# zyc00/Point-SAM

Hardware: AMD Instinct MI355X
Metric: point-clouds/sec (encode+1-prompt decode) (higher is better)
Workload: dtype f32 (fp32 in/out/accumulate; large GEMMs as row-scaled 2-way fp16 split x 3 MFMA products, fp32-grade error)

## Files before the change

point_sam_amd/build.py:

```python
import os
import subprocess
import sys
from concurrent.futures import ThreadPoolExecutor

CSRC = os.path.join(os.path.dirname(os.path.abspath(__file__)), "csrc")
LIB = os.path.join(CSRC, "libpointsam_hip.so")
HIPCC = os.environ.get("HIPCC", "/opt/rocm/bin/hipcc")
ARCH = "gfx950"
COMMON = ["--offload-arch=" + ARCH, "-O3", "-std=c++17", "-fPIC", "-fvisibility=hidden", "-Wall", "-Wno-unused-function"]
EXPERIMENTS = os.environ.get("PSAM_BUILD_EXPERIMENTS", "0") == "1"
SOURCES = [
    ("tokenizer.hip", ["-ffp-contract=off"]),
    ("gemm.hip", []),
    ("gemm_split.hip", []),
    ("gemm_f16x3p.hip", []),
    ("gemm_f16x3pp.hip", []),
    ("attention.hip", []),
    ("rowops.hip", []),
    ("blocks.hip", []),
    ("masks.hip", []),
    ("error.cpp", ["-x", "hip"]),
] + ([("experiments/gemm_f16x3q.hip", ["-I" + CSRC]), ("experiments/gemm_f16x3s.hip", ["-I" + CSRC]), ("experiments/gemm_f16x3c.hip", ["-I" + CSRC]),
        ("experiments/twoway.hip", ["-I" + CSRC])] if EXPERIMENTS else [])
if EXPERIMENTS:
    COMMON = COMMON + ["-DPSAM_BUILD_EXPERIMENTS"]
FLAGS_STAMP = os.path.join(CSRC, ".build_flags")
PROBE_SRC = os.path.join(CSRC, "probe", "mfma_probe.hip")
PROBE_LIB = os.path.join(CSRC, "probe", "libpsam_probe.so")


def _stale(out, deps):
    return not os.path.exists(out) or any(os.path.getmtime(d) > os.path.getmtime(out) for d in deps)


def build_library(force: bool = False, verbose: bool = False) -> str:
    hdrs = [os.path.join(CSRC, f) for f in sorted(os.listdir(CSRC)) if f.endswith(".h")]
    hdrs.append(os.path.join(os.path.dirname(os.path.dirname(CSRC)), "include", "pointsam_hip.h"))
    flags = " ".join(COMMON)
    if (open(FLAGS_STAMP).read() != flags) if os.path.exists(FLAGS_STAMP) else EXPERIMENTS:
        force = True
    jobs = []
    for src, extra in SOURCES:
        s = os.path.join(CSRC, src)
        o = os.path.join(CSRC, os.path.splitext(src)[0] + ".o")
        if force or _stale(o, [s, os.path.abspath(__file__)] + hdrs):
            jobs.append([HIPCC] + COMMON + extra + ["-c", s, "-o", o])
    def run(cmd):
        if verbose:
            print(" ".join(cmd), flush=True)
        r = subprocess.run(cmd, capture_output=True, text=True)
        if r.returncode != 0:
            raise RuntimeError("hipcc failed:\n" + " ".join(cmd) + "\n" + r.stderr)
        return r.stderr
    with ThreadPoolExecutor(max_workers=4) as ex:
        list(ex.map(run, jobs))
    objs = [os.path.join(CSRC, os.path.splitext(s)[0] + ".o") for s, _ in SOURCES]
    if force or jobs or _stale(LIB, objs):
        tmp = LIB + ".unlinted"
        run([HIPCC, "--offload-arch=" + ARCH, "-shared", "-fPIC", "-o", tmp] + objs)
        try:
            from . import isa_lint
        except ImportError:
            sys.path.insert(0, os.path.dirname(os.path.abspath(__file__)))
            import isa_lint
        bad = isa_lint.lint(tmp)
        if bad:
            os.replace(tmp, LIB + ".rejected")
            raise RuntimeError("libpointsam_hip.so contains packed-FP32 instructions with a non-uniform op_sel (see point_sam_amd/isa_lint.py):\n" +
                               "\n".join(f"  {k}: {i}" for k, i in bad))
        os.replace(tmp, LIB)
        with open(FLAGS_STAMP, "w") as f:
            f.write(flags)
    if force or _stale(PROBE_LIB, [PROBE_SRC]):
        run([HIPCC, "--offload-arch=" + ARCH, "-O3", "-std=c++17", "-fPIC", "-shared", "-o", PROBE_LIB, PROBE_SRC])
    return LIB


if __name__ == "__main__":
    print(build_library(force="--force" in sys.argv, verbose=True))
```

point_sam_amd/csrc/attention.hip:

```cpp
#include "common.h"
#include <math.h>
#include <utility>
#include <cstdlib>

typedef float f32x16 __attribute__((ext_vector_type(16)));
typedef float f32x4 __attribute__((ext_vector_type(4)));

constexpr int FA_BQ = 128;
constexpr int FA_BKV = 64;

struct FlashArgs {
    const float* q; const float* k; const float* v; float* o;
    int64_t ldq, ldk, ldv, ldo, sq, sk, sv, so;
    int H, Lq, Lk, B;
    float scale_log2e;
    const float* a_scale; float* o_scale; float k1, k2;
    int hd;
    int ksplit; float* sk_part; int* sk_count;
#ifdef PSAM_ATTN_ABLATE
    int abl;
#endif
};
#ifdef PSAM_ATTN_ABLATE
#define FA_ABL(bit) (p.abl & (bit))
// ... 336 lines not shown
        for (int s = 0; s < KSA; ++s)
#pragma unroll
            for (int e = 0; e < 2; ++e) {
                t[s][e] = (ok && s * 16 + h * 8 + e * 4 < hd) ? *reinterpret_cast<const f32x4*>(qp + s * 16 + e * 4) : f32x4{0.f, 0.f, 0.f, 0.f};
                amax = fmaxf(fmaxf(amax, fmaxf(fabsf(t[s][e][0]), fabsf(t[s][e][1]))), fmaxf(fabsf(t[s][e][2]), fabsf(t[s][e][3])));
            }
        amax = fmaxf(amax, __shfl_xor(amax, 32, 64));
        const float sq = f16_row_scale(amax);
        q_inv = fa_inv_pow2(sq);
#pragma unroll
        for (int s = 0; s < KSA; ++s) {
            unsigned hi[4], lo[4];
#pragma unroll
            for (int e = 0; e < 2; ++e) {
                fa_split2(fa_f32x2{t[s][e][0], t[s][e][1]} * sq, hi[2 * e], lo[2 * e]);
                fa_split2(fa_f32x2{t[s][e][2], t[s][e][3]} * sq, hi[2 * e + 1], lo[2 * e + 1]);
            }
            qh[s] = __builtin_bit_cast(fa_f16x8, fa_u32x4{hi[0], hi[1], hi[2], hi[3]});
            ql[s] = __builtin_bit_cast(fa_f16x8, fa_u32x4{lo[0], lo[1], lo[2], lo[3]});
        }
    }

    publish_max(0);
    __syncthreads();
    tile_scales(0, sk_cur, sv_cur);
    store_tile(0, sk_cur, sv_cur);
    __syncthreads();
    for (int t = t_first; t < ntiles; ++t) {
        const int buf = (t - t_first) & 1;
        const unsigned char* st_base = smem + buf * STAGE;
        if (t + 1 < ntiles && !FA_ABL(2)) load_tile((t + 1) * FA_BKV);
        const float c_s = p.scale_log2e * q_inv * fa_inv_pow2(sk_cur);
#pragma unroll
        for (int kt = 0; kt < FA_BKV / 32; ++kt) {
            const int key_base = t * FA_BKV + kt * 32;
            if (key_base >= p.Lk) break;
            f32x16 st;
#pragma unroll
            for (int r = 0; r < 16; ++r) st[r] = 0.f;
            const int krow = kt * 32 + r32;
            const unsigned char* kb = st_base + krow * KROW;
#pragma unroll
            for (int s = 0; s < KSA; ++s) {
                const int off = ((2 * s + h) ^ ((krow >> 1) & KSW)) << 4;
                const fa_f16x8 kh = *reinterpret_cast<const fa_f16x8*>(kb + off);
                const fa_f16x8 kl = *reinterpret_cast<const fa_f16x8*>(kb + KPLANE + off);
                if (FA_ABL(8)) { st[0] += (float)kh[0] + (float)kl[1]; continue; }
                st = __builtin_amdgcn_mfma_f32_32x32x16_f16(kh, ql[s], st, 0, 0, 0);
                st = __builtin_amdgcn_mfma_f32_32x32x16_f16(kl, qh[s], st, 0, 0, 0);
                st = __builtin_amdgcn_mfma_f32_32x32x16_f16(kh, qh[s], st, 0, 0, 0);
            }
            if (key_base + 32 > p.Lk) {
#pragma unroll
                for (int r = 0; r < 16; ++r)
                    if (key_base + (r & 3) + 8 * (r >> 2) + 4 * h >= p.Lk) st[r] = -INFINITY;
            }
            float mx = -INFINITY;
#pragma unroll
            for (int r = 0; r < 16; ++r) mx = fmaxf(mx, st[r]);
            mx = fmaxf(mx, __shfl_xor(mx, 32, 64)) * c_s;
            const float m_new = fmaxf(m_run, mx);
            const float alpha = __builtin_amdgcn_exp2f(m_run - m_new);
            const float m14 = m_new - 14.f;
            float ps = 0.f;
#pragma unroll
            for (int r = 0; r < 16; ++r) {
                st[r] = FA_ABL(4) ? __builtin_fmaf(st[r], c_s, -m14) : __builtin_amdgcn_exp2f(__builtin_fmaf(st[r], c_s, -m14));
                ps += st[r];
            }
            l_run = l_run * alpha + ps;
            m_run = m_new;
            const float fo = alpha * (sv_cur * fa_inv_pow2(sv_acc));
            sv_acc = sv_cur;
            if (__builtin_amdgcn_ballot_w64(fo != 1.f) != 0) {
#pragma unroll
                for (int d = 0; d < DT; ++d)
#pragma unroll
                    for (int r = 0; r < 16; ++r) oacc[d][r] *= fo;
            }
            fa_f16x8 ph[2], pl[2];
#pragma unroll
            for (int s2 = 0; s2 < 2; ++s2) {
                unsigned hi[4], lo[4];
#pragma unroll
                for (int e = 0; e < 4; ++e) {
                    if (FA_ABL(4)) { hi[e] = __builtin_bit_cast(unsigned, st[8 * s2 + 2 * e]); lo[e] = __builtin_bit_cast(unsigned, st[8 * s2 + 2 * e + 1]); }
                    else fa_split2(fa_f32x2{st[8 * s2 + 2 * e], st[8 * s2 + 2 * e + 1]}, hi[e], lo[e]);
                }
                ph[s2] = __builtin_bit_cast(fa_f16x8, fa_u32x4{hi[0], hi[1], hi[2], hi[3]});
                pl[s2] = __builtin_bit_cast(fa_f16x8, fa_u32x4{lo[0], lo[1], lo[2], lo[3]});
            }
#pragma unroll
            for (int s2 = 0; s2 < 2; ++s2)
#pragma unroll
                for (int d = 0; d < DTA; ++d) {
                    const int vrow = d * 32 + r32;
                    const unsigned char* vb = st_base + 2 * KPLANE + vrow * ROWB + (((kt * 4 + s2 * 2 + h) ^ ((vrow >> 1) & 7)) << 4);
                    const fa_f16x8 vh = *reinterpret_cast<const fa_f16x8*>(vb);
                    const fa_f16x8 vl = *reinterpret_cast<const fa_f16x8*>(vb + VPLANE);
                    if (FA_ABL(16)) { oacc[d][0] += (float)vh[0] + (float)vl[1] + (float)pl[s2][0] + (float)ph[s2][1]; continue; }
                    oacc[d] = __builtin_amdgcn_mfma_f32_32x32x16_f16(vh, pl[s2], oacc[d], 0, 0, 0);
                    oacc[d] = __builtin_amdgcn_mfma_f32_32x32x16_f16(vl, ph[s2], oacc[d], 0, 0, 0);
                    oacc[d] = __builtin_amdgcn_mfma_f32_32x32x16_f16(vh, ph[s2], oacc[d], 0, 0, 0);
                }
        }
        if (t + 1 < ntiles && !FA_ABL(1)) {
            publish_max(buf ^ 1);
            __syncthreads();
            tile_scales(buf ^ 1, sk_cur, sv_cur);
            store_tile(buf ^ 1, sk_cur, sv_cur);
        }
        if (!FA_ABL(32)) __syncthreads();
    }

    float l_tot = l_run + __shfl_xor(l_run, 32, 64);
    if (p.ksplit > 1) {
        constexpr int SC1 = 16, QUADS = DT * 4, SPLIT_BYTES = (QUADS * 256 + 128) * 16;
        const __amdgpu_buffer_rsrc_t rs = __builtin_amdgcn_make_buffer_rsrc((void*)(p.sk_part + (int64_t)bid * p.ksplit * (SPLIT_BYTES / 4)), 0, 0x7fffffff, 0x00020000);
        const float isv = fa_inv_pow2(sv_acc);
#pragma unroll
        for (int d = 0; d < DT; ++d)
#pragma unroll
            for (int r4 = 0; r4 < 4; ++r4) {
                const float a0 = oacc[d][4 * r4] * isv, a1 = oacc[d][4 * r4 + 1] * isv, a2 = oacc[d][4 * r4 + 2] * isv, a3 = oacc[d][4 * r4 + 3] * isv;
                const f32x4 vf = {a0, a1, a2, a3};
                __builtin_amdgcn_raw_buffer_store_b128(__builtin_bit_cast(fa_u32x4, vf), rs, split * SPLIT_BYTES + ((d * 4 + r4) * 256 + tid) * 16, 0, SC1);
            }
        {
            const fa_f32x2 ml = {m_run, l_tot};
            __builtin_amdgcn_raw_buffer_store_b64(__builtin_bit_cast(fa_u32x2, ml), rs, split * SPLIT_BYTES + QUADS * 256 * 16 + tid * 8, 0, SC1);
        }
        asm volatile("s_waitcnt vmcnt(0)" ::: "memory");
        __syncthreads();
        int* flag = reinterpret_cast<int*>(&smax[0][0][0]);
        if (tid == 0) *flag = (int)__hip_atomic_fetch_add(p.sk_count + bid, 1, __ATOMIC_RELAXED, __HIP_MEMORY_SCOPE_AGENT);
        __syncthreads();
        if (*flag != p.ksplit - 1) return;
        if (tid == 0) __hip_atomic_store(p.sk_count + bid, 0, __ATOMIC_RELAXED, __HIP_MEMORY_SCOPE_AGENT);
        float ms[4], ls[4], m_all = -INFINITY;
#pragma unroll
        for (int sp = 0; sp < 4; ++sp) {
            ms[sp] = -INFINITY; ls[sp] = 0.f;
            if (sp < p.ksplit) {
                const fa_f32x2 ml = __builtin_bit_cast(fa_f32x2, __builtin_amdgcn_raw_buffer_load_b64(rs, sp * SPLIT_BYTES + QUADS * 256 * 16 + tid * 8, 0, SC1));
                ms[sp] = ml[0]; ls[sp] = ml[1];
                m_all = fmaxf(m_all, ml[0]);
            }
        }
#pragma unroll
        for (int d = 0; d < DT; ++d)
#pragma unroll
            for (int r = 0; r < 16; ++r) oacc[d][r] = 0.f;
        l_tot = 0.f;
#pragma unroll
        for (int sp = 0; sp < 4; ++sp) {
            if (sp < p.ksplit) {
                const float w = __builtin_amdgcn_exp2f(ms[sp] - m_all);
                l_tot = __builtin_fmaf(w, ls[sp], l_tot);
#pragma unroll
                for (int d = 0; d < DT; ++d)
#pragma unroll
                    for (int r4 = 0; r4 < 4; ++r4) {
                        const f32x4 v = __builtin_bit_cast(f32x4, __builtin_amdgcn_raw_buffer_load_b128(rs, sp * SPLIT_BYTES + ((d * 4 + r4) * 256 + tid) * 16, 0, SC1));
#pragma unroll
                        for (int e = 0; e < 4; ++e) oacc[d][4 * r4 + e] = __builtin_fmaf(w, v[e], oacc[d][4 * r4 + e]);
                    }
            }
        }
        sv_acc = 1.f;
    }
    const float inv = fa_inv_pow2(sv_acc) / l_tot;
    const int qrow = q0 + r32;
    if (p.o_scale) {
        if (head == 0 && h == 0 && qrow < p.Lq) p.o_scale[(int64_t)b * p.Lq + qrow] = out_scale;
        float* op = p.o + b * p.so + (int64_t)(qrow < p.Lq ? qrow : 0) * p.ldo + head * hd;
#pragma unroll
        for (int d = 0; d < DT; ++d)
#pragma unroll
            for (int g = 0; g < 4; ++g) {
                const int d0 = d * 32 + 8 * g + 4 * h;
                unsigned h0, l0, h1, l1;
                fa_split2(fa_f32x2{oacc[d][4 * g] * inv, oacc[d][4 * g + 1] * inv} * out_scale, h0, l0);
                fa_split2(fa_f32x2{oacc[d][4 * g + 2] * inv, oacc[d][4 * g + 3] * inv} * out_scale, h1, l1);
                const unsigned r0 = __shfl_xor(h ? h0 : l0, 32, 64), r1 = __shfl_xor(h ? h1 : l1, 32, 64);
                if (qrow < p.Lq && d0 < hd) *reinterpret_cast<fa_u32x4*>(op + d0) = h ? fa_u32x4{r0, r1, l0, l1} : fa_u32x4{h0, h1, r0, r1};
            }
        return;
    }
    if (qrow < p.Lq) {
        float* op = p.o + b * p.so + (int64_t)qrow * p.ldo + head * hd;
#pragma unroll
        for (int d = 0; d < DT; ++d)
#pragma unroll
            for (int g = 0; g < 4; ++g) {
                const int d0 = d * 32 + 8 * g + 4 * h;
                f32x4 o4 = {oacc[d][4 * g] * inv, oacc[d][4 * g + 1] * inv, oacc[d][4 * g + 2] * inv, oacc[d][4 * g + 3] * inv};
                if (d0 < hd) *reinterpret_cast<f32x4*>(op + d0) = o4;
            }
    }
}

constexpr int64_t FA_SK_MAX_UNITS = PSAM_CNT_ATTN_N;
static int g_fa_keysplit = -1;
static bool fa_keysplit_enabled() {
    if (g_fa_keysplit >= 0) return g_fa_keysplit != 0;
    static int on = -1;
    if (on < 0) { const char* e = getenv("PSAM_ATTN_KEYSPLIT"); on = e ? (atoi(e) != 0) : 1; }
    return on != 0;
}
PSAM_API void psam_attention_f16x3_force_keysplit(int32_t mode) { g_fa_keysplit = mode; }
static bool fa_full_width() {
    static int on = -1;
    if (on < 0) { const char* e = getenv("PSAM_ATTN_FULL_WIDTH"); on = e ? (atoi(e) != 0) : 0; }
    return on != 0;
}
static int fa_keysplit_factor(int32_t B, int32_t H, int32_t Lq, int32_t Lk, int32_t hd, int32_t max_keysplit) {
    if (B <= 0 || H <= 0 || Lq <= 0 || Lk <= 0 || hd <= 64) return 1;
    const int64_t units = (int64_t)psam_cdiv(Lq, FA_BQ) * H * B;
    int dev = 0, ncu = 256;
    if (hipGetDevice(&dev) != hipSuccess || hipDeviceGetAttribute(&ncu, hipDeviceAttributeMultiprocessorCount, dev) != hipSuccess || ncu <= 0) ncu = 256;
    const int ntiles = (int)psam_cdiv(Lk, FA_BKV);
    int ks = fa_keysplit_enabled() ? (int)(ncu / units) : 1;
    if (ks > 4) ks = 4;
    if (ks > max_keysplit) ks = max_keysplit;
    if (ks > ntiles / 2) ks = ntiles / 2;
    return (ks > 1 && units <= FA_SK_MAX_UNITS) ? ks : 1;
}
static int64_t fa_split_bytes(int32_t hd) { return ((int64_t)((hd == 64 ? 64 : 128) / 32) * 4 * 256 + 128) * 16; }
PSAM_API size_t psam_attention_f16x3_keysplit_ws_bytes(int32_t B, int32_t H, int32_t Lq, int32_t Lk, int32_t hd, int32_t max_keysplit) {
    const int ks = fa_keysplit_factor(B, H, Lq, Lk, hd, max_keysplit);
    return ks > 1 ? (size_t)((int64_t)psam_cdiv(Lq, FA_BQ) * H * B * ks * fa_split_bytes(hd)) : 0;
}

PSAM_API int32_t psam_attention_f16x3_ex2(const float* q, int64_t ldq, int64_t sq, const float* k, int64_t ldk, int64_t sk, const float* v, int64_t ldv,
                                          int64_t sv, float* o, int64_t ldo, int64_t so, int32_t B, int32_t H, int32_t Lq, int32_t Lk, int32_t hd,
                                          float scale, const float* a_scale, float k1, float k2, float* o_scale, int32_t max_keysplit, void* ks_ws,
                                          size_t ks_ws_bytes, int32_t* counters, hipStream_t stream) {
    PSAM_REQUIRE(q && k && v && o, PSAM_EINVAL, "psam_attention_f16x3: null pointer");
    PSAM_REQUIRE((a_scale == nullptr) == (o_scale == nullptr), PSAM_EINVAL, "psam_attention_f16x3: packed output needs both a_scale and o_scale");
    PSAM_REQUIRE(!o_scale || ((ldo & 7) == 0 && ((uintptr_t)o & 31) == 0 && (so & 7) == 0 && Lq == Lk), PSAM_EINVAL,
                 "psam_attention_f16x3: packed output needs 32-byte aligned rows and self-attention (Lq == Lk)");
    PSAM_REQUIRE(B > 0 && H > 0 && Lq > 0 && Lk > 0, PSAM_EINVAL, "psam_attention_f16x3: bad shape");
    PSAM_REQUIRE((int64_t)psam_cdiv(Lq, FA_BQ) * H * B < ((int64_t)1 << 31), PSAM_EINVAL, "psam_attention_f16x3: too many workgroups");
    PSAM_REQUIRE(((ldq | ldk | ldv | ldo | sq | sk | sv | so) & 3) == 0 && (((uintptr_t)q | (uintptr_t)k | (uintptr_t)v | (uintptr_t)o) & 15) == 0,
                 PSAM_EALIGN, "psam_attention_f16x3: strides must be multiples of 4 floats and pointers 16-byte aligned");
    PSAM_REQUIRE((int64_t)Lk * ldk < ((int64_t)1 << 29) && (int64_t)Lk * ldv < ((int64_t)1 << 29), PSAM_EINVAL,
                 "psam_attention_f16x3: one (batch) K/V slice must span < 2 GiB (32-bit buffer offsets)");
    FlashArgs p;
    p.q = q; p.k = k; p.v = v; p.o = o;
    p.ldq = ldq; p.ldk = ldk; p.ldv = ldv; p.ldo = ldo; p.sq = sq; p.sk = sk; p.sv = sv; p.so = so;
    p.H = H; p.Lq = Lq; p.Lk = Lk; p.B = B;
    p.scale_log2e = scale * 1.4426950408889634f;
    p.a_scale = a_scale; p.o_scale = o_scale; p.k1 = k1; p.k2 = k2; p.hd = hd;
#ifdef PSAM_ATTN_ABLATE
    p.abl = g_attn_abl;
#endif
    p.ksplit = 1; p.sk_part = nullptr; p.sk_count = nullptr;
    const int64_t units = (int64_t)psam_cdiv(Lq, FA_BQ) * H * B;
    if (ks_ws && counters) {
        int ks = fa_keysplit_factor(B, H, Lq, Lk, hd, max_keysplit);
        while (ks > 1 && (size_t)(units * ks * fa_split_bytes(hd)) > ks_ws_bytes) --ks;
        if (ks > 1) {
            PSAM_REQUIRE(((uintptr_t)ks_ws & 15) == 0, PSAM_EALIGN, "psam_attention_f16x3: ks_ws must be 16-byte aligned");
            p.ksplit = ks; p.sk_part = static_cast<float*>(ks_ws); p.sk_count = counters + PSAM_CNT_ATTN;
        }
    }
    const dim3 grid((unsigned)(units * p.ksplit)), block(256);
    if (hd == 64) hipLaunchKernelGGL((flash_attn_f16x3_kernel<64>), grid, block, 0, stream, p);
    else if (hd > 64 && hd <= 96 && (hd & 7) == 0 && !fa_full_width()) hipLaunchKernelGGL((flash_attn_f16x3_kernel<128, 96>), grid, block, 0, stream, p);
    else if (hd > 64 && hd <= 128 && (hd & 7) == 0) hipLaunchKernelGGL((flash_attn_f16x3_kernel<128>), grid, block, 0, stream, p);
    else {
        psam_set_error("psam_attention_f16x3: head_dim must be 64 or a multiple of 8 in (64, 128]");
        return PSAM_EINVAL;
    }
    return psam_launch_status("psam_attention_f16x3: launch failed");
}

PSAM_API int32_t psam_attention_f16x3_ex(const float* q, int64_t ldq, int64_t sq, const float* k, int64_t ldk, int64_t sk, const float* v, int64_t ldv,
                                         int64_t sv, float* o, int64_t ldo, int64_t so, int32_t B, int32_t H, int32_t Lq, int32_t Lk, int32_t hd,
                                         float scale, const float* a_scale, float k1, float k2, float* o_scale, hipStream_t stream) {
    return psam_attention_f16x3_ex2(q, ldq, sq, k, ldk, sk, v, ldv, sv, o, ldo, so, B, H, Lq, Lk, hd, scale, a_scale, k1, k2, o_scale, 1, nullptr, 0, nullptr, stream);
}

PSAM_API int32_t psam_attention_f16x3(const float* q, int64_t ldq, int64_t sq, const float* k, int64_t ldk, int64_t sk, const float* v, int64_t ldv,
                                      int64_t sv, float* o, int64_t ldo, int64_t so, int32_t B, int32_t H, int32_t Lq, int32_t Lk, int32_t hd,
                                      float scale, hipStream_t stream) {
    return psam_attention_f16x3_ex(q, ldq, sq, k, ldk, sk, v, ldv, sv, o, ldo, so, B, H, Lq, Lk, hd, scale, nullptr, 0.f, 0.f, nullptr, stream);
}

struct PackedAttnArgs {
    const unsigned char* qkv;
    const float* sc;
    float* o; float* o_scale;
    int64_t ld, ldo;
    int H, L, B, D;
    float scale_log2e, v_bound;
#ifdef PSAM_ATTN_ABLATE
    int abl;
#endif
};

typedef short fa_s16x4 __attribute__((__vector_size__(4 * sizeof(short))));
typedef short fa_s16x8 __attribute__((ext_vector_type(8)));
__device__ __forceinline__ fa_s16x4 fa_ds_read_tr16(const unsigned char* lds_ptr) {
#if defined(__HIP_DEVICE_COMPILE__)
    return __builtin_amdgcn_ds_read_tr16_b64_v4i16((__attribute__((address_space(3))) fa_s16x4*)(lds_ptr));
#else
    (void)lds_ptr; return fa_s16x4{0, 0, 0, 0};
#endif
}

#if defined(__HIP_DEVICE_COMPILE__)
#define FA_DMA16(rsrc, dst, voff, soff) __builtin_amdgcn_raw_ptr_buffer_load_lds(rsrc, (__attribute__((address_space(3))) void*)(dst), 16, voff, soff, 0, 0)
#else
#define FA_DMA16(rsrc, dst, voff, soff) ((void)(rsrc), (void)(dst), (void)(voff), (void)(soff))
#endif

constexpr int PA_BQ = 256;
#ifndef PA_PRIO
#define PA_PRIO 1
#endif
constexpr int PA_TILE = FA_BKV * 256;

template <int NW, int RING = 3, int QB = 1>
__global__ __launch_bounds__(64 * NW, RING == 2 ? 2 : 1) void flash_attn_packed_kernel(const PackedAttnArgs p) {
    constexpr int HD = 64, KS = 4, DT = 2, ROWB = 256;
    static_assert(RING == 3 || (RING == 2 && NW == 4), "ring of three tiles, or two tiles with four waves (two workgroups per CU)");
    constexpr int BQ = NW * 32 * QB, NPC = 32 / NW;
    static_assert(QB == 1 || (QB == 2 && NW == 4 && RING == 3), "two query blocks per wave: four waves, three-tile ring");
    static_assert(NW == 8 || NW == 4, "waves per workgroup");
    extern __shared__ __attribute__((aligned(16))) unsigned char smem[];
    const int tid = threadIdx.x, lane = tid & 63;
    const int wave = __builtin_amdgcn_readfirstlane(tid >> 6);
    const int r32 = lane & 31, h = lane >> 5;
    const int nq = (p.L + BQ - 1) / BQ, HB = p.H * p.B;
    int qb, hb;
    if ((HB & 7) == 0) { const int id = blockIdx.x, grp = id / (8 * nq), r = id - grp * 8 * nq; hb = grp * 8 + (r & 7); qb = r >> 3; }
    else { qb = blockIdx.x % nq; hb = blockIdx.x / nq; }
    const int head = hb % p.H, b = hb / p.H;
    const int64_t rowb = p.ld * 4;
    const unsigned char* base = p.qkv + (int64_t)b * p.L * rowb + (int64_t)head * HD * 4;
    const float s_u = p.sc[(int64_t)b * p.L];

    const int nt = (p.L + FA_BKV - 1) / FA_BKV;
    const __amdgpu_buffer_rsrc_t rs = __builtin_amdgcn_make_buffer_rsrc((void*)base, 0, 0x7fffffff, 0x00020000);
    int dvoff[NPC];
    int dkey[NPC];
#pragma unroll
    for (int i = 0; i < NPC; ++i) {
        const int pc = wave * NPC + i;
        const bool isv = pc >= 16;
        const int row = (pc & 15) * 4 + (lane >> 4), slot = lane & 15;
        const int chunk = slot ^ (isv ? ((row & 1) | ((row & 2) << 2)) : (row & 15));
        dkey[i] = row;
        dvoff[i] = (isv ? 2 : 1) * p.D * 4 + chunk * 16;
    }
    auto issue_tile = [&](int t, int buf) {
#pragma unroll
        for (int i = 0; i < NPC; ++i) {
            const int pc = wave * NPC + i;
            int key = t * FA_BKV + dkey[i];
            key = key < p.L ? key : p.L - 1;
            unsigned char* dst = smem + buf * 2 * PA_TILE + (pc >= 16 ? PA_TILE : 0) + (pc & 15) * 1024;
            FA_DMA16(rs, dst, (int)((int64_t)key * rowb) + dvoff[i], 0);
        }
    };
    issue_tile(0, 0);
    if (RING == 3 && nt > 1) issue_tile(1, 1);

    const int q0 = qb * BQ + wave * 32 * QB;
    int qrow[QB];
    fa_f16x8 qh[QB][KS], ql[QB][KS];
#pragma unroll
    for (int u = 0; u < QB; ++u) {
        qrow[u] = q0 + 32 * u + r32;
        const unsigned char* qp = base + (int64_t)(qrow[u] < p.L ? qrow[u] : p.L - 1) * rowb;
#pragma unroll
        for (int s = 0; s < KS; ++s) {
            qh[u][s] = *reinterpret_cast<const fa_f16x8*>(qp + (2 * s + h) * 32);
            ql[u][s] = *reinterpret_cast<const fa_f16x8*>(qp + (2 * s + h) * 32 + 16);
        }
    }
    const float inv_su = fa_inv_pow2(s_u);
    const float c_s = p.scale_log2e * inv_su * inv_su;

    f32x16 oacc[QB][DT];
    float m_run[QB], l_run[QB];
#pragma unroll
    for (int u = 0; u < QB; ++u) {
        m_run[u] = -INFINITY; l_run[u] = 0.f;
#pragma unroll
        for (int d = 0; d < DT; ++d)
#pragma unroll
            for (int r = 0; r < 16; ++r) oacc[u][d][r] = 0.f;
    }

    const int tr_key = (lane & 15) >> 2, tr_d = ((lane >> 4) & 1) * 16 + 4 * (lane & 3);
    const int tr_sw = (tr_key & 1) | ((tr_key & 2) << 2);

    if (PA_PRIO && NW == 8 && wave >= 4) __builtin_amdgcn_s_setprio(1);
    int buf = 0;
    for (int t = 0; t < (FA_ABL(128) ? 0 : nt); ++t) {
        if (RING == 3 && t + 1 < nt) asm volatile("s_waitcnt vmcnt(%0)" ::"n"(NPC) : "memory");
        else asm volatile("s_waitcnt vmcnt(0)" ::: "memory");
        if (!FA_ABL(2)) __builtin_amdgcn_s_barrier();
        if (RING == 3) { if (t + 2 < nt && !FA_ABL(1)) issue_tile(t + 2, buf == 0 ? 2 : buf - 1); }
        else if (t + 1 < nt && !FA_ABL(1)) issue_tile(t + 1, buf ^ 1);
        const unsigned char* kt0 = smem + buf * 2 * PA_TILE;
        const unsigned char* vt0 = kt0 + PA_TILE;
        f32x16 st[QB][2];
#pragma unroll
        for (int kt = 0; kt < 2; ++kt) {
            f32x16 sa[QB], sb[QB];
#pragma unroll
            for (int u = 0; u < QB; ++u)
#pragma unroll
                for (int r = 0; r < 16; ++r) { sa[u][r] = 0.f; sb[u][r] = 0.f; }
            const int krow = kt * 32 + r32;
            const unsigned char* kb = kt0 + krow * ROWB;
#pragma unroll
            for (int sp = 0; sp < KS / 2; ++sp) {
                fa_f16x8 kh[2], kl[2];
#pragma unroll
                for (int u = 0; u < 2; ++u) {
                    const int c = 2 * (2 * (sp + 2 * u) + h);
                    kh[u] = *reinterpret_cast<const fa_f16x8*>(kb + (((c) ^ (krow & 15)) << 4));
                    kl[u] = *reinterpret_cast<const fa_f16x8*>(kb + (((c + 1) ^ (krow & 15)) << 4));
                }
#pragma unroll
                for (int u = 0; u < QB; ++u) {
                    sa[u] = __builtin_amdgcn_mfma_f32_32x32x16_f16(kh[0], ql[u][sp], sa[u], 0, 0, 0);
                    sb[u] = __builtin_amdgcn_mfma_f32_32x32x16_f16(kh[1], ql[u][sp + 2], sb[u], 0, 0, 0);
                }
#pragma unroll
                for (int u = 0; u < QB; ++u) {
                    sa[u] = __builtin_amdgcn_mfma_f32_32x32x16_f16(kl[0], qh[u][sp], sa[u], 0, 0, 0);
                    sb[u] = __builtin_amdgcn_mfma_f32_32x32x16_f16(kl[1], qh[u][sp + 2], sb[u], 0, 0, 0);
                }
#pragma unroll
                for (int u = 0; u < QB; ++u) {
                    sa[u] = __builtin_amdgcn_mfma_f32_32x32x16_f16(kh[0], qh[u][sp], sa[u], 0, 0, 0);
                    sb[u] = __builtin_amdgcn_mfma_f32_32x32x16_f16(kh[1], qh[u][sp + 2], sb[u], 0, 0, 0);
                }
            }
#pragma unroll
            for (int u = 0; u < QB; ++u)
#pragma unroll
                for (int r = 0; r < 16; ++r) st[u][kt][r] = sa[u][r] + sb[u][r];
        }
#pragma unroll
        for (int kt = 0; kt < 2; ++kt) {
            const int key_base = t * FA_BKV + kt * 32;
            fa_f16x8 vh[2][DT], vl[2][DT];
#pragma unroll
            for (int s2 = 0; s2 < 2; ++s2)
#pragma unroll
                for (int d = 0; d < DT; ++d) {
                    const int kbase = kt * 32 + 16 * s2 + 4 * h;
                    const int ch = d * 32 + tr_d;
                    const int chunk = 2 * (ch >> 3), inb = (ch & 7) * 2;
                    const unsigned char* a0 = vt0 + (kbase + tr_key) * ROWB + inb;
                    const unsigned char* a1 = a0 + 8 * ROWB;
                    const fa_s16x4 h0 = fa_ds_read_tr16(a0 + (((chunk) ^ tr_sw) << 4)), h1 = fa_ds_read_tr16(a1 + (((chunk) ^ tr_sw) << 4));
                    const fa_s16x4 l0 = fa_ds_read_tr16(a0 + (((chunk + 1) ^ tr_sw) << 4)), l1 = fa_ds_read_tr16(a1 + (((chunk + 1) ^ tr_sw) << 4));
                    vh[s2][d] = __builtin_bit_cast(fa_f16x8, fa_s16x8{h0[0], h0[1], h0[2], h0[3], h1[0], h1[1], h1[2], h1[3]});
                    vl[s2][d] = __builtin_bit_cast(fa_f16x8, fa_s16x8{l0[0], l0[1], l0[2], l0[3], l1[0], l1[1], l1[2], l1[3]});
                }
#pragma unroll
            for (int u = 0; u < QB; ++u) {
            if (key_base + 32 > p.L) {
#pragma unroll
                for (int r = 0; r < 16; ++r)
                    if (key_base + (r & 3) + 8 * (r >> 2) + 4 * h >= p.L) st[u][kt][r] = -INFINITY;
            }
            float mxa = fmaxf(fmaxf(st[u][kt][0], st[u][kt][1]), fmaxf(st[u][kt][2], st[u][kt][3])), mxb = fmaxf(fmaxf(st[u][kt][4], st[u][kt][5]), fmaxf(st[u][kt][6], st[u][kt][7]));
            float mxc = fmaxf(fmaxf(st[u][kt][8], st[u][kt][9]), fmaxf(st[u][kt][10], st[u][kt][11])), mxd = fmaxf(fmaxf(st[u][kt][12], st[u][kt][13]), fmaxf(st[u][kt][14], st[u][kt][15]));
            float mx = fmaxf(fmaxf(mxa, mxb), fmaxf(mxc, mxd));
            mx = fmaxf(mx, __shfl_xor(mx, 32, 64)) * c_s;
            const float m_new = fmaxf(m_run[u], mx);
            const float alpha = __builtin_amdgcn_exp2f(m_run[u] - m_new);
            const float m14 = m_new - 14.f;
            float psum[4] = {0.f, 0.f, 0.f, 0.f};
#pragma unroll
            for (int r = 0; r < 16; ++r) {
                st[u][kt][r] = __builtin_amdgcn_exp2f(__builtin_fmaf(st[u][kt][r], c_s, -m14));
                psum[r & 3] += st[u][kt][r];
            }
            l_run[u] = l_run[u] * alpha + ((psum[0] + psum[1]) + (psum[2] + psum[3]));
            m_run[u] = m_new;
            if (__builtin_amdgcn_ballot_w64(alpha != 1.f) != 0) {
#pragma unroll
                for (int d = 0; d < DT; ++d)
#pragma unroll
                    for (int r = 0; r < 16; ++r) oacc[u][d][r] *= alpha;
            }
#pragma unroll
            for (int s2 = 0; s2 < 2; ++s2) {
                unsigned hi[4], lo[4];
#pragma unroll
                for (int e = 0; e < 4; ++e) fa_split2(fa_f32x2{st[u][kt][8 * s2 + 2 * e], st[u][kt][8 * s2 + 2 * e + 1]}, hi[e], lo[e]);
                const fa_f16x8 ph = __builtin_bit_cast(fa_f16x8, fa_u32x4{hi[0], hi[1], hi[2], hi[3]});
                const fa_f16x8 pl = __builtin_bit_cast(fa_f16x8, fa_u32x4{lo[0], lo[1], lo[2], lo[3]});
#pragma unroll
                for (int d = 0; d < DT; ++d) oacc[u][d] = __builtin_amdgcn_mfma_f32_32x32x16_f16(vh[s2][d], pl, oacc[u][d], 0, 0, 0);
#pragma unroll
                for (int d = 0; d < DT; ++d) oacc[u][d] = __builtin_amdgcn_mfma_f32_32x32x16_f16(vl[s2][d], ph, oacc[u][d], 0, 0, 0);
#pragma unroll
                for (int d = 0; d < DT; ++d) oacc[u][d] = __builtin_amdgcn_mfma_f32_32x32x16_f16(vh[s2][d], ph, oacc[u][d], 0, 0, 0);
            }
            }
        }
        buf = RING == 2 ? (buf ^ 1) : (buf == 2 ? 0 : buf + 1);
    }

    if (FA_ABL(256)) { if (l_run[0] == 123.f) p.o_scale[0] = oacc[0][0][0] + oacc[0][1][5]; return; }
    const float out_scale = f16_row_scale(p.v_bound);
#pragma unroll
    for (int u = 0; u < QB; ++u) {
        const float l_tot = l_run[u] + __shfl_xor(l_run[u], 32, 64);
        const float inv = inv_su / l_tot;
        if (head == 0 && h == 0 && qrow[u] < p.L) p.o_scale[(int64_t)b * p.L + qrow[u]] = out_scale;
        float* op = p.o + ((int64_t)b * p.L + (qrow[u] < p.L ? qrow[u] : 0)) * p.ldo + head * HD;
#pragma unroll
        for (int d = 0; d < DT; ++d)
#pragma unroll
            for (int g = 0; g < 4; ++g) {
                const int d0 = d * 32 + 8 * g + 4 * h;
                unsigned h0, l0, h1, l1;
                fa_split2(fa_f32x2{oacc[u][d][4 * g] * inv, oacc[u][d][4 * g + 1] * inv} * out_scale, h0, l0);
                fa_split2(fa_f32x2{oacc[u][d][4 * g + 2] * inv, oacc[u][d][4 * g + 3] * inv} * out_scale, h1, l1);
                const unsigned r0 = __shfl_xor(h ? h0 : l0, 32, 64), r1 = __shfl_xor(h ? h1 : l1, 32, 64);
                if (qrow[u] < p.L) *reinterpret_cast<fa_u32x4*>(op + d0) = h ? fa_u32x4{r0, r1, l0, l1} : fa_u32x4{h0, h1, r0, r1};
            }
    }
}

static int g_attn_variant = -1;
static int attn_variant_env() {
    static int v = -2;
    if (v == -2) { const char* e = getenv("PSAM_ATTN_VARIANT"); v = e ? atoi(e) : 1; }
    return v;
}
PSAM_API void psam_attention_packed_force_variant(int32_t v) { g_attn_variant = v; }

PSAM_API int32_t psam_attention_packed(const void* qkv, int64_t ld, const float* sc, float* o, int64_t ldo, float* o_scale, int32_t B, int32_t H,
                                       int32_t L, int32_t hd, float scale, float v_bound, hipStream_t stream) {
    PSAM_REQUIRE(qkv && sc && o && o_scale, PSAM_EINVAL, "psam_attention_packed: null pointer");
    PSAM_REQUIRE(B > 0 && H > 0 && L > 0 && hd == 64, PSAM_EINVAL, "psam_attention_packed: bad shape (head_dim 64)");
    PSAM_REQUIRE(ld >= 3 * (int64_t)H * hd && (ld & 7) == 0 && (ldo & 7) == 0 && ldo >= (int64_t)H * hd && (((uintptr_t)qkv | (uintptr_t)o) & 31) == 0, PSAM_EALIGN,
                 "psam_attention_packed: packed rows must be 32-byte aligned, ld >= 3 H hd");
    PSAM_REQUIRE((int64_t)L * ld * 4 < ((int64_t)1 << 31), PSAM_EINVAL, "psam_attention_packed: one cloud's qkv slice must span < 2 GiB (32-bit buffer offsets)");
    PSAM_REQUIRE(v_bound > 0.f && (int64_t)psam_cdiv(L, PA_BQ) * H * B < ((int64_t)1 << 31), PSAM_EINVAL, "psam_attention_packed: bad bound / too many workgroups");
    PackedAttnArgs p;
    p.qkv = (const unsigned char*)qkv; p.sc = sc; p.o = o; p.o_scale = o_scale; p.ld = ld; p.ldo = ldo; p.H = H; p.L = L; p.B = B; p.D = H * hd;
    p.scale_log2e = scale * 1.4426950408889634f; p.v_bound = v_bound;
#ifdef PSAM_ATTN_ABLATE
    p.abl = g_attn_abl;
#endif
    constexpr int lds = 3 * 2 * PA_TILE;
    static unsigned long long attr_done = 0;
    int dev = 0, ncu = 256;
    PSAM_REQUIRE(hipGetDevice(&dev) == hipSuccess, PSAM_EINVAL, "psam_attention_packed: no device");
    {
        const unsigned long long bit = 1ull << (dev & 63);
        if (!(__atomic_load_n(&attr_done, __ATOMIC_ACQUIRE) & bit)) {
            PSAM_REQUIRE(hipFuncSetAttribute(reinterpret_cast<const void*>(&flash_attn_packed_kernel<8>), hipFuncAttributeMaxDynamicSharedMemorySize, lds) == hipSuccess &&
                         hipFuncSetAttribute(reinterpret_cast<const void*>(&flash_attn_packed_kernel<4>), hipFuncAttributeMaxDynamicSharedMemorySize, lds) == hipSuccess &&
                         hipFuncSetAttribute(reinterpret_cast<const void*>(&flash_attn_packed_kernel<4, 2>), hipFuncAttributeMaxDynamicSharedMemorySize, 2 * 2 * PA_TILE) == hipSuccess
#ifdef PSAM_BUILD_EXPERIMENTS
                         && hipFuncSetAttribute(reinterpret_cast<const void*>(&flash_attn_packed_kernel<4, 3, 2>), hipFuncAttributeMaxDynamicSharedMemorySize, lds) == hipSuccess
#endif
                         ,
                         PSAM_EINVAL, "psam_attention_packed: cannot reserve LDS");
            __atomic_fetch_or(&attr_done, bit, __ATOMIC_RELEASE);
        }
    }
    static int force_nw = -1;
    if (force_nw < 0) { const char* e = getenv("PSAM_ATTN_PACKED_NW"); force_nw = e ? atoi(e) : 0; }
    if (hipDeviceGetAttribute(&ncu, hipDeviceAttributeMultiprocessorCount, dev) != hipSuccess || ncu <= 0) ncu = 256;
    const int64_t wg8 = (int64_t)psam_cdiv(L, PA_BQ) * H * B;
    const bool small = force_nw ? force_nw == 4 : (wg8 < ncu && L > PA_BQ / 2);
    const int variant = g_attn_variant >= 0 ? g_attn_variant : attn_variant_env();
    const int64_t wg4 = (int64_t)psam_cdiv(L, PA_BQ / 2) * H * B;
#ifdef PSAM_BUILD_EXPERIMENTS
    if (variant == 2 && !force_nw && L > PA_BQ / 2) {
        hipLaunchKernelGGL((flash_attn_packed_kernel<4, 3, 2>), dim3((unsigned)wg8), dim3(256), lds, stream, p);
        return psam_launch_status("psam_attention_packed: launch failed");
    }
#endif
    if (variant == 1 && !force_nw && L > PA_BQ / 2 && wg4 <= (int64_t)4 * ncu) {
        hipLaunchKernelGGL((flash_attn_packed_kernel<4, 2>), dim3((unsigned)wg4), dim3(256), 2 * 2 * PA_TILE, stream, p);
        if (psam_ablate_repeat() & 1) hipLaunchKernelGGL((flash_attn_packed_kernel<4, 2>), dim3((unsigned)wg4), dim3(256), 2 * 2 * PA_TILE, stream, p);
        return psam_launch_status("psam_attention_packed: launch failed");
    }
    if (small) hipLaunchKernelGGL(flash_attn_packed_kernel<4>, dim3((unsigned)(psam_cdiv(L, PA_BQ / 2) * H * B)), dim3(256), lds, stream, p);
    else hipLaunchKernelGGL(flash_attn_packed_kernel<8>, dim3((unsigned)wg8), dim3(512), lds, stream, p);
    return psam_launch_status("psam_attention_packed: launch failed");
}
```

point_sam_amd/isa_lint.py:

```python
import os
import re
import shutil
import subprocess
import sys
import tempfile

LLVM = os.environ.get("PSAM_LLVM_BIN", "/opt/rocm/lib/llvm/bin")
_PK = re.compile(r"^\s*(v_pk_(?:mul|add|fma)_f32)\s+(.*?)(?:\s*//.*)?$")
_SEL = re.compile(r"\bop_sel:\[([01](?:,[01])+)\]")


def hazardous(instruction: str) -> bool:
    m = _PK.match(instruction)
    if not m:
        return False
    s = _SEL.search(m.group(2))
    return bool(s) and len(set(s.group(1).split(","))) > 1


def device_disassembly(lib: str):
    objdump = os.path.join(LLVM, "llvm-objdump")
    with tempfile.TemporaryDirectory() as tmp:
        copy = os.path.join(tmp, os.path.basename(lib))
        shutil.copyfile(lib, copy)
        subprocess.run([objdump, "--offloading", copy], check=True, capture_output=True)
        objs = sorted(f for f in os.listdir(tmp) if "amdgcn" in f)
        if not objs:
            raise RuntimeError(f"{lib}: no device code objects found")
        for f in objs:
            r = subprocess.run([objdump, "-d", os.path.join(tmp, f)], check=True, capture_output=True, text=True)
            kernel = "?"
            for line in r.stdout.splitlines():
                k = re.match(r"^[0-9a-f]+ <(.*)>:", line)
                if k:
                    kernel = k.group(1)
                elif line.startswith(("\t", " ")):
                    yield kernel, line.strip()


def lint(lib: str):
    return [(k, i.split("//")[0].strip()) for k, i in device_disassembly(lib) if hazardous(i)]


def main(argv):
    lib = argv[1] if len(argv) > 1 else os.path.join(os.path.dirname(os.path.abspath(__file__)), "csrc", "libpointsam_hip.so")
    bad = lint(lib)
    for k, i in bad:
        print(f"{k}: {i}")
    print(f"{lib}: {len(bad)} packed-FP32 instruction(s) with a non-uniform op_sel")
    return 1 if bad else 0


if __name__ == "__main__":
    sys.exit(main(sys.argv))
```

Before: 787.6.

## Hoist V transposed-read addressing, prefetch V earlier, streamline DMA offsets in packed attention

Reworks the packed flash-attention inner loop. Per-lane LDS addresses for the transposed V reads are precomputed, and the reads use inline asm with immediate offsets, issued ahead of the softmax with an explicit lgkmcnt wait just before the MFMAs. DMA tile addressing moves the per-tile offset into the scalar soffset and clamps only on the last partial tile. The row-max reduction uses v_max3, the fp16 split uses an FMA with a scalar -1 (fa_split2m), and SLP vectorization is disabled for this file. The aim is fewer VALU address and max instructions and better overlap of LDS latency with the softmax math, at the cost of asm-level control that the compiler can no longer schedule around.

Result: no change. 790.0, median of 6 (+0.3%).

```diff
diff --git a/point_sam_amd/build.py b/point_sam_amd/build.py
--- a/point_sam_amd/build.py
+++ b/point_sam_amd/build.py
@@ -15,7 +15,7 @@
     ("gemm_split.hip", []),
     ("gemm_f16x3p.hip", []),
     ("gemm_f16x3pp.hip", []),
-    ("attention.hip", []),
+    ("attention.hip", ["-fno-slp-vectorize"]),
     ("rowops.hip", []),
     ("blocks.hip", []),
     ("masks.hip", []),
diff --git a/point_sam_amd/csrc/attention.hip b/point_sam_amd/csrc/attention.hip
--- a/point_sam_amd/csrc/attention.hip
+++ b/point_sam_amd/csrc/attention.hip
@@ -662,12 +662,41 @@
 
 typedef short fa_s16x4 __attribute__((__vector_size__(4 * sizeof(short))));
 typedef short fa_s16x8 __attribute__((ext_vector_type(8)));
-__device__ __forceinline__ fa_s16x4 fa_ds_read_tr16(const unsigned char* lds_ptr) {
+template <int OFF>
+__device__ __forceinline__ fa_s16x4 fa_ds_read_tr16(unsigned lds_addr) {
+    static_assert(OFF >= 0 && OFF < 65536, "ds_read offset field: 16 bits");
+    fa_s16x4 r;
 #if defined(__HIP_DEVICE_COMPILE__)
-    return __builtin_amdgcn_ds_read_tr16_b64_v4i16((__attribute__((address_space(3))) fa_s16x4*)(lds_ptr));
+    asm volatile("ds_read_b64_tr_b16 %0, %1 offset:%2" : "=v"(r) : "v"(lds_addr), "n"(OFF) : "memory");
 #else
-    (void)lds_ptr; return fa_s16x4{0, 0, 0, 0};
-#endif
+    (void)lds_addr; r = fa_s16x4{0, 0, 0, 0};
+#endif
+    return r;
+}
+#if defined(__HIP_DEVICE_COMPILE__)
+#define FA_TR_WAIT8(a) asm volatile("s_waitcnt lgkmcnt(0)" : "+v"((a)[0]), "+v"((a)[1]), "+v"((a)[2]), "+v"((a)[3]), "+v"((a)[4]), "+v"((a)[5]), "+v"((a)[6]), "+v"((a)[7]))
+#else
+#define FA_TR_WAIT8(a) ((void)(a))
+#endif
+__device__ __forceinline__ float fa_max3(float a, float b, float c) {
+#if defined(__HIP_DEVICE_COMPILE__)
+    float d; asm("v_max3_f32 %0, %1, %2, %3" : "=v"(d) : "v"(a), "v"(b), "v"(c)); return d;
+#else
+    return fmaxf(fmaxf(a, b), c);
+#endif
+}
+__device__ __forceinline__ float fa_max2(float a, float b) {
+#if defined(__HIP_DEVICE_COMPILE__)
+    float d; asm("v_max_f32 %0, %1, %2" : "=v"(d) : "v"(a), "v"(b)); return d;
+#else
+    return fmaxf(a, b);
+#endif
+}
+__device__ __forceinline__ void fa_split2m(const float x0, const float x1, const float m1, unsigned& hi, unsigned& lo) {
+    const fa_f16x2 h = __builtin_convertvector(fa_f32x2{x0, x1}, fa_f16x2);
+    const fa_f16x2 l = {(_Float16)__builtin_fmaf((float)h[0], m1, x0), (_Float16)__builtin_fmaf((float)h[1], m1, x1)};
+    hi = __builtin_bit_cast(unsigned, h);
+    lo = __builtin_bit_cast(unsigned, l);
 }
 
 #if defined(__HIP_DEVICE_COMPILE__)
@@ -713,16 +742,25 @@
         const int row = (pc & 15) * 4 + (lane >> 4), slot = lane & 15;
         const int chunk = slot ^ (isv ? ((row & 1) | ((row & 2) << 2)) : (row & 15));
         dkey[i] = row;
-        dvoff[i] = (isv ? 2 : 1) * p.D * 4 + chunk * 16;
+        dvoff[i] = row * (int)rowb + (isv ? 2 : 1) * p.D * 4 + chunk * 16;
     }
     auto issue_tile = [&](int t, int buf) {
-#pragma unroll
-        for (int i = 0; i < NPC; ++i) {
-            const int pc = wave * NPC + i;
-            int key = t * FA_BKV + dkey[i];
-            key = key < p.L ? key : p.L - 1;
-            unsigned char* dst = smem + buf * 2 * PA_TILE + (pc >= 16 ? PA_TILE : 0) + (pc & 15) * 1024;
-            FA_DMA16(rs, dst, (int)((int64_t)key * rowb) + dvoff[i], 0);
+        const int soff = t * FA_BKV * (int)rowb;
+        if (t == nt - 1 && (p.L & (FA_BKV - 1))) {
+#pragma unroll
+            for (int i = 0; i < NPC; ++i) {
+                const int pc = wave * NPC + i;
+                const int over = t * FA_BKV + dkey[i] - (p.L - 1);
+                unsigned char* dst = smem + buf * 2 * PA_TILE + (pc >= 16 ? PA_TILE : 0) + (pc & 15) * 1024;
+                FA_DMA16(rs, dst, dvoff[i] - (over > 0 ? over : 0) * (int)rowb, soff);
+            }
+        } else {
+#pragma unroll
+            for (int i = 0; i < NPC; ++i) {
+                const int pc = wave * NPC + i;
+                unsigned char* dst = smem + buf * 2 * PA_TILE + (pc >= 16 ? PA_TILE : 0) + (pc & 15) * 1024;
+                FA_DMA16(rs, dst, dvoff[i], soff);
+            }
         }
     };
     issue_tile(0, 0);
@@ -759,6 +797,20 @@
     const int tr_sw = (tr_key & 1) | ((tr_key & 2) << 2);
 
     if (PA_PRIO && NW == 8 && wave >= 4) __builtin_amdgcn_s_setprio(1);
+    unsigned tr_lane[DT][2];
+#pragma unroll
+    for (int d = 0; d < DT; ++d)
+#pragma unroll
+        for (int pl = 0; pl < 2; ++pl) {
+            const int ch = d * 32 + tr_d, chunk = 2 * (ch >> 3) + pl, inb = (ch & 7) * 2;
+            tr_lane[d][pl] = (unsigned)(size_t)((__attribute__((address_space(3))) unsigned char*)smem) + PA_TILE + (4 * h + tr_key) * ROWB + inb + ((chunk ^ tr_sw) << 4);
+        }
+#pragma unroll
+    for (int u = 0; u < QB; ++u)
+#pragma unroll
+        for (int s = 0; s < KS; ++s) asm volatile("" ::"v"(qh[u][s]), "v"(ql[u][s]));
+    float m1 = -1.f;
+    asm("" : "+s"(m1));
     int buf = 0;
     for (int t = 0; t < (FA_ABL(128) ? 0 : nt); ++t) {
         if (RING == 3 && t + 1 < nt) asm volatile("s_waitcnt vmcnt(%0)" ::"n"(NPC) : "memory");
@@ -767,7 +819,7 @@
         if (RING == 3) { if (t + 2 < nt && !FA_ABL(1)) issue_tile(t + 2, buf == 0 ? 2 : buf - 1); }
         else if (t + 1 < nt && !FA_ABL(1)) issue_tile(t + 1, buf ^ 1);
         const unsigned char* kt0 = smem + buf * 2 * PA_TILE;
-        const unsigned char* vt0 = kt0 + PA_TILE;
+        const unsigned tr_buf = buf * 2 * PA_TILE;
         f32x16 st[QB][2];
 #pragma unroll
         for (int kt = 0; kt < 2; ++kt) {
@@ -811,21 +863,22 @@
 #pragma unroll
         for (int kt = 0; kt < 2; ++kt) {
             const int key_base = t * FA_BKV + kt * 32;
-            fa_f16x8 vh[2][DT], vl[2][DT];
-#pragma unroll
-            for (int s2 = 0; s2 < 2; ++s2)
-#pragma unroll
-                for (int d = 0; d < DT; ++d) {
-                    const int kbase = kt * 32 + 16 * s2 + 4 * h;
-                    const int ch = d * 32 + tr_d;
-                    const int chunk = 2 * (ch >> 3), inb = (ch & 7) * 2;
-                    const unsigned char* a0 = vt0 + (kbase + tr_key) * ROWB + inb;
-                    const unsigned char* a1 = a0 + 8 * ROWB;
-                    const fa_s16x4 h0 = fa_ds_read_tr16(a0 + (((chunk) ^ tr_sw) << 4)), h1 = fa_ds_read_tr16(a1 + (((chunk) ^ tr_sw) << 4));
-                    const fa_s16x4 l0 = fa_ds_read_tr16(a0 + (((chunk + 1) ^ tr_sw) << 4)), l1 = fa_ds_read_tr16(a1 + (((chunk + 1) ^ tr_sw) << 4));
-                    vh[s2][d] = __builtin_bit_cast(fa_f16x8, fa_s16x8{h0[0], h0[1], h0[2], h0[3], h1[0], h1[1], h1[2], h1[3]});
-                    vl[s2][d] = __builtin_bit_cast(fa_f16x8, fa_s16x8{l0[0], l0[1], l0[2], l0[3], l1[0], l1[1], l1[2], l1[3]});
+            fa_s16x4 vr[2][8];
+#pragma unroll
+            for (int d = 0; d < DT; ++d) {
+                const unsigned ah = tr_lane[d][0] + tr_buf, al = tr_lane[d][1] + tr_buf;
+                if (kt == 0) {
+                    vr[0][4 * d + 0] = fa_ds_read_tr16<0 * ROWB>(ah); vr[0][4 * d + 1] = fa_ds_read_tr16<8 * ROWB>(ah);
+                    vr[0][4 * d + 2] = fa_ds_read_tr16<0 * ROWB>(al); vr[0][4 * d + 3] = fa_ds_read_tr16<8 * ROWB>(al);
+                    vr[1][4 * d + 0] = fa_ds_read_tr16<16 * ROWB>(ah); vr[1][4 * d + 1] = fa_ds_read_tr16<24 * ROWB>(ah);
+                    vr[1][4 * d + 2] = fa_ds_read_tr16<16 * ROWB>(al); vr[1][4 * d + 3] = fa_ds_read_tr16<24 * ROWB>(al);
+                } else {
+                    vr[0][4 * d + 0] = fa_ds_read_tr16<32 * ROWB>(ah); vr[0][4 * d + 1] = fa_ds_read_tr16<40 * ROWB>(ah);
+                    vr[0][4 * d + 2] = fa_ds_read_tr16<32 * ROWB>(al); vr[0][4 * d + 3] = fa_ds_read_tr16<40 * ROWB>(al);
+                    vr[1][4 * d + 0] = fa_ds_read_tr16<48 * ROWB>(ah); vr[1][4 * d + 1] = fa_ds_read_tr16<56 * ROWB>(ah);
+                    vr[1][4 * d + 2] = fa_ds_read_tr16<48 * ROWB>(al); vr[1][4 * d + 3] = fa_ds_read_tr16<56 * ROWB>(al);
                 }
+            }
 #pragma unroll
             for (int u = 0; u < QB; ++u) {
             if (key_base + 32 > p.L) {
@@ -833,10 +886,11 @@
                 for (int r = 0; r < 16; ++r)
                     if (key_base + (r & 3) + 8 * (r >> 2) + 4 * h >= p.L) st[u][kt][r] = -INFINITY;
             }
-            float mxa = fmaxf(fmaxf(st[u][kt][0], st[u][kt][1]), fmaxf(st[u][kt][2], st[u][kt][3])), mxb = fmaxf(fmaxf(st[u][kt][4], st[u][kt][5]), fmaxf(st[u][kt][6], st[u][kt][7]));
-            float mxc = fmaxf(fmaxf(st[u][kt][8], st[u][kt][9]), fmaxf(st[u][kt][10], st[u][kt][11])), mxd = fmaxf(fmaxf(st[u][kt][12], st[u][kt][13]), fmaxf(st[u][kt][14], st[u][kt][15]));
-            float mx = fmaxf(fmaxf(mxa, mxb), fmaxf(mxc, mxd));
-            mx = fmaxf(mx, __shfl_xor(mx, 32, 64)) * c_s;
+#define SV(i) st[u][kt][i]
+            float mx = fa_max3(fa_max3(fa_max3(SV(0), SV(1), SV(2)), fa_max3(SV(3), SV(4), SV(5)), fa_max3(SV(6), SV(7), SV(8))),
+                               fa_max3(SV(9), SV(10), SV(11)), fa_max3(SV(12), SV(13), fa_max2(SV(14), SV(15))));
+#undef SV
+            mx = fa_max2(mx, __shfl_xor(mx, 32, 64)) * c_s;
             const float m_new = fmaxf(m_run[u], mx);
             const float alpha = __builtin_amdgcn_exp2f(m_run[u] - m_new);
             const float m14 = m_new - 14.f;
@@ -858,15 +912,23 @@
             for (int s2 = 0; s2 < 2; ++s2) {
                 unsigned hi[4], lo[4];
 #pragma unroll
-                for (int e = 0; e < 4; ++e) fa_split2(fa_f32x2{st[u][kt][8 * s2 + 2 * e], st[u][kt][8 * s2 + 2 * e + 1]}, hi[e], lo[e]);
+                for (int e = 0; e < 4; ++e) fa_split2m(st[u][kt][8 * s2 + 2 * e], st[u][kt][8 * s2 + 2 * e + 1], m1, hi[e], lo[e]);
                 const fa_f16x8 ph = __builtin_bit_cast(fa_f16x8, fa_u32x4{hi[0], hi[1], hi[2], hi[3]});
                 const fa_f16x8 pl = __builtin_bit_cast(fa_f16x8, fa_u32x4{lo[0], lo[1], lo[2], lo[3]});
-#pragma unroll
-                for (int d = 0; d < DT; ++d) oacc[u][d] = __builtin_amdgcn_mfma_f32_32x32x16_f16(vh[s2][d], pl, oacc[u][d], 0, 0, 0);
-#pragma unroll
-                for (int d = 0; d < DT; ++d) oacc[u][d] = __builtin_amdgcn_mfma_f32_32x32x16_f16(vl[s2][d], ph, oacc[u][d], 0, 0, 0);
-#pragma unroll
-                for (int d = 0; d < DT; ++d) oacc[u][d] = __builtin_amdgcn_mfma_f32_32x32x16_f16(vh[s2][d], ph, oacc[u][d], 0, 0, 0);
+                if (u == 0) FA_TR_WAIT8(vr[s2]);
+                fa_f16x8 vh[DT], vl[DT];
+#pragma unroll
+                for (int d = 0; d < DT; ++d) {
+                    const fa_s16x4 h0 = vr[s2][4 * d], h1 = vr[s2][4 * d + 1], l0 = vr[s2][4 * d + 2], l1 = vr[s2][4 * d + 3];
+                    vh[d] = __builtin_bit_cast(fa_f16x8, fa_s16x8{h0[0], h0[1], h0[2], h0[3], h1[0], h1[1], h1[2], h1[3]});
+                    vl[d] = __builtin_bit_cast(fa_f16x8, fa_s16x8{l0[0], l0[1], l0[2], l0[3], l1[0], l1[1], l1[2], l1[3]});
+                }
+#pragma unroll
+                for (int d = 0; d < DT; ++d) oacc[u][d] = __builtin_amdgcn_mfma_f32_32x32x16_f16(vh[d], pl, oacc[u][d], 0, 0, 0);
+#pragma unroll
+                for (int d = 0; d < DT; ++d) oacc[u][d] = __builtin_amdgcn_mfma_f32_32x32x16_f16(vl[d], ph, oacc[u][d], 0, 0, 0);
+#pragma unroll
+                for (int d = 0; d < DT; ++d) oacc[u][d] = __builtin_amdgcn_mfma_f32_32x32x16_f16(vh[d], ph, oacc[u][d], 0, 0, 0);
             }
             }
         }
@@ -887,8 +949,8 @@
             for (int g = 0; g < 4; ++g) {
                 const int d0 = d * 32 + 8 * g + 4 * h;
                 unsigned h0, l0, h1, l1;
-                fa_split2(fa_f32x2{oacc[u][d][4 * g] * inv, oacc[u][d][4 * g + 1] * inv} * out_scale, h0, l0);
-                fa_split2(fa_f32x2{oacc[u][d][4 * g + 2] * inv, oacc[u][d][4 * g + 3] * inv} * out_scale, h1, l1);
+                fa_split2m(oacc[u][d][4 * g] * inv * out_scale, oacc[u][d][4 * g + 1] * inv * out_scale, m1, h0, l0);
+                fa_split2m(oacc[u][d][4 * g + 2] * inv * out_scale, oacc[u][d][4 * g + 3] * inv * out_scale, m1, h1, l1);
                 const unsigned r0 = __shfl_xor(h ? h0 : l0, 32, 64), r1 = __shfl_xor(h ? h1 : l1, 32, 64);
                 if (qrow[u] < p.L) *reinterpret_cast<fa_u32x4*>(op + d0) = h ? fa_u32x4{r0, r1, l0, l1} : fa_u32x4{h0, h1, r0, r1};
             }
diff --git a/point_sam_amd/isa_lint.py b/point_sam_amd/isa_lint.py
--- a/point_sam_amd/isa_lint.py
+++ b/point_sam_amd/isa_lint.py
@@ -38,6 +38,61 @@
                     yield kernel, line.strip()
 
 
+_ADDR = re.compile(r"//\s*([0-9A-Fa-f]+):")
+_TARGET = re.compile(r"<[^>]*\+0x([0-9a-fA-F]+)>\s*$")
+_LDS_DMA = re.compile(r"^buffer_load_dwordx4\b.*\blds\b")
+
+
+def kernel_instructions(lib: str, name_part: str):
+    out, start = {}, {}
+    for k, line in device_disassembly(lib):
+        if name_part not in k:
+            continue
+        a = _ADDR.search(line)
+        if not a:
+            continue
+        addr = int(a.group(1), 16)
+        start.setdefault(k, addr)
+        text = line.split("//")[0].strip()
+        t = _TARGET.search(line) if re.match(r"s_c?branch", text) else None
+        out.setdefault(k, []).append((addr - start[k], text, int(t.group(1), 16) if t else None))
+    return out
+
+
+def dma_tile_loops(instructions):
+    offs = [o for o, _, _ in instructions]
+    spans = set()
+    for i, (o, _, tgt) in enumerate(instructions):
+        if tgt is not None and tgt <= o and tgt in offs:
+            j = offs.index(tgt)
+            body = [t for _, t, _ in instructions[j:i + 1]]
+            if any(t.startswith("v_mfma") for t in body) and any(_LDS_DMA.match(t) for t in body):
+                spans.add((j, i))
+    first = {}
+    for j, i in spans:
+        first[j] = max(first.get(j, i), i)
+    spans = sorted(first.items())
+    inner = [(j, i) for j, i in spans if not any((j2, i2) != (j, i) and j <= j2 and i2 <= i for j2, i2 in spans)]
+    return [[t for _, t, _ in instructions[j:i + 1]] for j, i in inner]
+
+
+def unbarriered_vmcnt_waits(body):
+    bad = []
+    for i, t in enumerate(body):
+        if t.startswith("s_waitcnt") and "vmcnt" in t:
+            for u in body[i + 1:]:
+                if u.startswith("s_barrier"):
+                    break
+                if u.startswith("v_mfma") or u.startswith("ds_read"):
+                    bad.append(t)
+                    break
+    return bad
+
+
+def packed_fp32(body):
+    return [t for t in body if _PK.match(t)]
+
+
 def lint(lib: str):
     return [(k, i.split("//")[0].strip()) for k, i in device_disassembly(lib) if hazardous(i)]
 
```
